# aujxn/faer-amg

Measured on AMD Instinct MI355X. Metric: V-cycles/s + fine-level SpMV GB/s vs HBM peak, 3D 7-pt Laplacian 256³, higher is better.
Workload: dtype f64

## Files before the change

faer-amg_amd/csrc/capi.cpp:

```cpp
#include <atomic>
#include <cmath>
#include <cstring>
#include <string>

#include "handles.hpp"
#include "solve.hpp"

using namespace famg;

namespace {
thread_local std::string g_last_error;
}

amg_status famg::set_last_error(amg_status s, const char *msg) {
    g_last_error = msg;
    return s;
}

namespace {
amg_linop *box(LinOpPtr p) { return new amg_linop{std::move(p)}; }

LinOp &need(const amg_linop *h) {
    FAMG_REQUIRE(h && h->op, AMG_ERR_INVALID, "null amg_linop handle");
    return *h->op;
}

CsrPtr need_csr(const amg_linop *h) {
    need(h);
    auto p = std::dynamic_pointer_cast<CsrOp>(h->op);
    FAMG_REQUIRE(p, AMG_ERR_INVALID, "operator is not a CSR matrix");
    return p;
}

std::shared_ptr<MultigridOp> need_mg(const amg_linop *h) {
    need(h);
    auto p = std::dynamic_pointer_cast<MultigridOp>(h->op);
    FAMG_REQUIRE(p, AMG_ERR_INVALID, "operator is not a multigrid");
    return p;
}

amg_ctx *ctx_of(const LinOp &op) {
    return reinterpret_cast<amg_ctx *>(op.ctx);
}

template <typename F>
void for_columns(LinOp &op, double *out, int64_t ld_out, const double *rhs, int64_t ld_rhs,
                 int64_t k, amg_mem mem, int64_t out_rows, int64_t rhs_rows, F &&f) {
    FAMG_REQUIRE(k >= 0, AMG_ERR_INVALID, "negative column count");
    if (k == 0) return;
    FAMG_REQUIRE(out && rhs, AMG_ERR_INVALID, "null vector");
    FAMG_REQUIRE(ld_out >= out_rows && ld_rhs >= rhs_rows, AMG_ERR_INVALID, "leading dimension too small");
    Ctx &ctx = *op.ctx;
    ctx.set_device();
    if (mem == AMG_MEM_DEVICE) {
        for (int64_t c = 0; c < k; c++) f(out + c * ld_out, rhs + c * ld_rhs);
        return;
    }
    FAMG_REQUIRE(mem == AMG_MEM_HOST, AMG_ERR_INVALID, "bad amg_mem");
    amg_ctx *ac = ctx_of(op);
    if (ac->stage_in.size() < (size_t)rhs_rows) ac->stage_in.resize(rhs_rows);
    if (ac->stage_out.size() < (size_t)out_rows) ac->stage_out.resize(out_rows);
    for (int64_t c = 0; c < k; c++) {
        FAMG_CHECK_HIP(hipMemcpyAsync(ac->stage_in.get(), rhs + c * ld_rhs, rhs_rows * sizeof(double),
                                      hipMemcpyHostToDevice, ctx.stream));
        f(ac->stage_out.get(), ac->stage_in.get());
        FAMG_CHECK_HIP(hipMemcpyAsync(out + c * ld_out, ac->stage_out.get(), out_rows * sizeof(double),
                                      hipMemcpyDeviceToHost, ctx.stream));
        FAMG_CHECK_HIP(hipStreamSynchronize(ctx.stream));
    }
}

}

namespace famg {
void export_plan(const std::vector<LaunchRec> &plan, amg_launch_rec *recs, int64_t cap, int64_t *count) {
    *count = (int64_t)plan.size();
    if (!recs) return;
    for (int64_t i = 0; i < std::min<int64_t>(cap, (int64_t)plan.size()); i++) {
        const LaunchRec &r = plan[i];
        amg_launch_rec &o = recs[i];
        o.level = r.level;
        o.role = r.role;
        o.kernel = r.kernel;
        o.mode = r.mode;
        o.rows = r.rows;
        o.bytes = r.bytes;
        o.csr_bytes = r.csr_bytes;
        std::memset(o.name, 0, sizeof(o.name));
        std::strncpy(o.name, r.name, sizeof(o.name) - 1);
    }
}
}

namespace famg {
static std::atomic<int64_t> g_flag_val[FLAG_COUNT] = {
    {(int64_t)env_is_one("FAMG_FOLD_XSCS")},
    {(int64_t)env_not_zero("FAMG_DIA_DK")},
    {[] {
        const int64_t w = env_int("FAMG_VEC_WPR", 0);
        return (w == 1 || w == 2 || w == 4) ? w : (int64_t)0;
    }()},
    {env_int("FAMG_GTX_TIME", 2)},
    {env_int("FAMG_SGS27_MARCH", 1)},
    {env_int("FAMG_XS_PIPE", 2)},
    {env_int("FAMG_BSR_KERNEL", 0)},
    {env_int("FAMG_BSR_LONG", 48)},
    {env_int("FAMG_DIA7_RP", 0)},
    {env_int("FAMG_FINE_FUSE", 1)},
    {env_int("FAMG_DENSE_TAIL", 4096)},
    {env_int("FAMG_BLOCK_CYCLE", 1)},
    {env_int("FAMG_BLOCK_SMOOTHER_COLS", 1)}};
static std::atomic<uint64_t> g_flag_gen{0};
int64_t flag(FlagId f) { return g_flag_val[f].load(std::memory_order_relaxed); }
void set_flag(FlagId f, int64_t v) {
    g_flag_val[f].store(v);
    g_flag_gen.fetch_add(1);
}
uint64_t flags_generation() { return g_flag_gen.load(); }
}

extern "C" {

const char *amg_last_error(void) { return g_last_error.c_str(); }
const char *amg_version(void) { return "faer-amg_amd 0.1.0 (gfx950)"; }

amg_status amg_ctx_create(int device, void *hip_stream, amg_ctx **out) {
    return guard([&] {
        FAMG_REQUIRE(out, AMG_ERR_INVALID, "null output pointer");
        int ndev = 0;
        FAMG_CHECK_HIP(hipGetDeviceCount(&ndev));
        FAMG_REQUIRE(device >= 0 && device < ndev, AMG_ERR_INVALID, "device index out of range");
        auto *c = new amg_ctx();
        c->ctx.device = device;
        try {
            c->ctx.set_device();
            if (hip_stream) {
                c->ctx.stream = static_cast<hipStream_t>(hip_stream);
            } else {
                FAMG_CHECK_HIP(hipStreamCreateWithFlags(&c->ctx.stream, hipStreamNonBlocking));
                c->ctx.own_stream = true;
            }
            hipDeviceProp_t prop;
            FAMG_CHECK_HIP(hipGetDeviceProperties(&prop, device));
            c->ctx.num_cus = prop.multiProcessorCount;
        } catch (...) {
            delete c;
            throw;
        }
        *out = c;
    });
}

amg_status amg_ctx_destroy(amg_ctx *ctx) {
    return guard([&] {
        if (!ctx) return;
        ctx->ctx.set_device();
        if (ctx->ctx.stream) (void)hipStreamSynchronize(ctx->ctx.stream);
        delete ctx;
    });
}

amg_status amg_ctx_synchronize(amg_ctx *ctx) {
    return guard([&] {
        FAMG_REQUIRE(ctx, AMG_ERR_INVALID, "null context");
        ctx->ctx.set_device();
        FAMG_CHECK_HIP(hipStreamSynchronize(ctx->ctx.stream));
    });
}

amg_status amg_ctx_stream(amg_ctx *ctx, void **hip_stream) {
    return guard([&] {
        FAMG_REQUIRE(ctx && hip_stream, AMG_ERR_INVALID, "null argument");
        *hip_stream = ctx->ctx.stream;
    });
}

amg_status amg_ctx_join_stream(amg_ctx *ctx, void *other, int32_t ctx_waits) {
    return guard([&] {
        FAMG_REQUIRE(ctx, AMG_ERR_INVALID, "null context");
        hipStream_t o = static_cast<hipStream_t>(other);
        if (o == ctx->ctx.stream) return;
        ctx->ctx.set_device();
        if (!ctx->join_event) FAMG_CHECK_HIP(hipEventCreateWithFlags(&ctx->join_event, hipEventDisableTiming));
        if (ctx_waits) {
            FAMG_CHECK_HIP(hipEventRecord(ctx->join_event, o));
            FAMG_CHECK_HIP(hipStreamWaitEvent(ctx->ctx.stream, ctx->join_event, 0));
        } else {
            FAMG_CHECK_HIP(hipEventRecord(ctx->join_event, ctx->ctx.stream));
            FAMG_CHECK_HIP(hipStreamWaitEvent(o, ctx->join_event, 0));
        }
    });
}

amg_status amg_set_alloc_policy(int32_t policy) {
    return guard([&] {
        FAMG_REQUIRE(policy == 0 || policy == 1, AMG_ERR_INVALID, "policy must be 0 or 1");
        FAMG_REQUIRE(policy == 0 || g_alloc_experiment > 0, AMG_ERR_UNSUPPORTED,
                     "contiguous allocations read stale data across kernels on gfx950 (DESIGN.md 3)");
        g_alloc_policy = policy;
    });
}

amg_status amg_set_value_codes(int32_t enable) {
    return guard([&] {
        FAMG_REQUIRE(enable >= 0 && enable <= 2, AMG_ERR_INVALID, "enable must be 0, 1 or 2");
        g_value_codes = enable;
    });
}

amg_status amg_set_sgs_fused(int32_t enable) {
    return guard([&] {
        FAMG_REQUIRE(enable >= 0 && enable <= 2, AMG_ERR_INVALID, "enable must be 0, 1 or 2");
        g_sgs_fused = enable;
    });
}

amg_status amg_sgs_fused(const amg_linop *op, int32_t *fused) {
    return guard([&] {
        FAMG_REQUIRE(fused, AMG_ERR_INVALID, "null output");
        auto p = std::dynamic_pointer_cast<SgsOp>(need(op).shared_from_this());
        FAMG_REQUIRE(p, AMG_ERR_INVALID, "operator is not an SGS smoother");
        *fused = p->fused27 ? 1 : 0;
    });
}

amg_status amg_set_spmv_format(int32_t policy) {
    return guard([&] {
        FAMG_REQUIRE(policy >= 0 && policy <= 3, AMG_ERR_INVALID, "policy must be 0..3");
        g_spmv_format_policy = policy;
    });
}


amg_status amg_csr_create(amg_ctx *ctx, int64_t nrows, int64_t ncols, const int64_t *rowptr,
                          const int64_t *colidx, const double *vals, amg_linop **out) {
    return guard([&] {
        FAMG_REQUIRE(ctx && out, AMG_ERR_INVALID, "null argument");
        FAMG_REQUIRE(nrows >= 0 && ncols >= 0, AMG_ERR_INVALID, "negative dimension");
        ctx->ctx.set_device();
        auto p = make_csr(&ctx->ctx);
        csr_from_host(p->m, &ctx->ctx, nrows, ncols, rowptr, colidx, vals);
        p->nrows = nrows;
        p->ncols = ncols;
        *out = box(p);
    });
}

__attribute__((visibility("default"))) amg_status amg_csr_create_device_i32(
    amg_ctx *ctx, int64_t nrows, int64_t ncols, const int32_t *rowptr, const int32_t *colidx,
    const double *vals, amg_linop **out) {
    return guard([&] {
        FAMG_REQUIRE(ctx && out && rowptr, AMG_ERR_INVALID, "null argument");
        ctx->ctx.set_device();
        hipStream_t s = ctx->ctx.stream;
        std::vector<int32_t> rp32(nrows + 1);
        FAMG_CHECK_HIP(hipMemcpyAsync(rp32.data(), rowptr, (nrows + 1) * sizeof(int32_t), hipMemcpyDeviceToHost, s));
        FAMG_CHECK_HIP(hipStreamSynchronize(s));
        std::vector<int64_t> rp(rp32.begin(), rp32.end());
        const int64_t nnz = rp[nrows];
        auto p = make_csr(&ctx->ctx);
        csr_alloc(p->m, &ctx->ctx, nrows, ncols, nnz);
        FAMG_CHECK_HIP(hipMemcpyAsync(p->m.rp64.get(), rp.data(), (nrows + 1) * sizeof(int64_t), hipMemcpyHostToDevice, s));
        if (nnz) {
            FAMG_CHECK_HIP(hipMemcpyAsync(p->m.col.get(), colidx, nnz * sizeof(int32_t), hipMemcpyDeviceToDevice, s));
// ... 911 lines not shown
```

faer-amg_amd/csrc/common.hpp:

```cpp
#pragma once

#include <hip/hip_runtime.h>

#include <cstdint>
#include <cstdio>
#include <cstdlib>
#include <memory>
#include <stdexcept>
#include <string>
#include <vector>

#include "../../include/amg.h"

namespace famg {

struct AmgError : std::runtime_error {
    amg_status status;
    AmgError(amg_status s, const std::string &msg) : std::runtime_error(msg), status(s) {}
};

[[noreturn]] inline void fail(amg_status s, const std::string &msg) { throw AmgError(s, msg); }

#define FAMG_CHECK_HIP(expr)                                                               \
    do {                                                                                   \
        hipError_t e_ = (expr);                                                            \
        if (e_ != hipSuccess) {                                                            \
            ::famg::fail(e_ == hipErrorOutOfMemory ? AMG_ERR_OOM : AMG_ERR_HIP,            \
                         std::string(#expr) + ": " + hipGetErrorString(e_) + " at " +      \
                             __FILE__ + ":" + std::to_string(__LINE__));                   \
        }                                                                                  \
    } while (0)

#define FAMG_REQUIRE(cond, status, msg)                                                    \
    do {                                                                                   \
        if (!(cond)) ::famg::fail(status, msg);                                            \
    } while (0)

extern int g_alloc_policy;

extern bool g_alloc_debug;

extern int g_alloc_experiment;
inline void *dev_alloc(size_t bytes) {
    void *p = nullptr;
    const bool large = bytes >= (size_t(16) << 20);
    if (g_alloc_policy == 1 && large) {
        if (hipExtMallocWithFlags(&p, bytes, hipDeviceMallocContiguous) == hipSuccess && p) {
            if (g_alloc_debug) fprintf(stderr, "famg alloc contiguous %p %zu\n", p, bytes);
            if (g_alloc_experiment == 2) FAMG_CHECK_HIP(hipDeviceSynchronize());
            return p;
        }
        (void)hipGetLastError();
        p = nullptr;
    }
    FAMG_CHECK_HIP(hipMalloc(&p, bytes));
    if (g_alloc_debug && large) fprintf(stderr, "famg alloc plain %p %zu\n", p, bytes);
    return p;
}

template <typename T> class DevBuf {
  public:
    DevBuf() = default;
    explicit DevBuf(size_t n) { resize(n); }
    DevBuf(const DevBuf &) = delete;
    DevBuf &operator=(const DevBuf &) = delete;
    DevBuf(DevBuf &&o) noexcept : p_(o.p_), n_(o.n_) { o.p_ = nullptr; o.n_ = 0; }
    DevBuf &operator=(DevBuf &&o) noexcept {
        if (this != &o) { release(); p_ = o.p_; n_ = o.n_; o.p_ = nullptr; o.n_ = 0; }
        return *this;
    }
    ~DevBuf() { release(); }
    void resize(size_t n, size_t pad = 0) {
        release();
        if (n + pad) p_ = static_cast<T *>(dev_alloc((n + pad) * sizeof(T)));
        n_ = n;
    }
    void release() {
        if (p_) (void)hipFree(p_);
        p_ = nullptr;
        n_ = 0;
    }
    T *get() const { return p_; }
    size_t size() const { return n_; }
    size_t bytes() const { return n_ * sizeof(T); }

  private:
    T *p_ = nullptr;
    size_t n_ = 0;
};

struct Ctx {
    int device = 0;
    hipStream_t stream = nullptr;
    bool own_stream = false;
    int num_cus = 256;
    DevBuf<double> red_partials;
    DevBuf<double> red_result;
    double *host_red = nullptr;
    void set_device() const { FAMG_CHECK_HIP(hipSetDevice(device)); }
    ~Ctx();
};

inline int64_t ceil_div(int64_t a, int64_t b) { return (a + b - 1) / b; }

inline bool env_is_one(const char *name) {
    const char *e = getenv(name);
    return e && e[0] == '1';
}
inline bool env_not_zero(const char *name) {
    const char *e = getenv(name);
    return !(e && e[0] == '0');
}
inline int64_t env_int(const char *name, int64_t dflt) {
    const char *e = getenv(name);
    return e ? atoll(e) : dflt;
}
inline int env_char(const char *name) {
    const char *e = getenv(name);
    return e ? (int)(unsigned char)e[0] : -1;
}

enum FlagId : int { FLAG_FOLD_XSCS = 0, FLAG_DIA_DK = 1, FLAG_VEC_WPR = 2, FLAG_GTX_TIME = 3, FLAG_SGS27_MARCH = 4, FLAG_XS_PIPE = 5,
              FLAG_BSR_KERNEL = 6, FLAG_BSR_LONG = 7,
              FLAG_DIA7_RP = 8, FLAG_FINE_FUSE = 9, FLAG_DENSE_TAIL = 10, FLAG_BLOCK_CYCLE = 11,
              FLAG_BLOCK_SMOOTHER_COLS = 12, FLAG_COUNT = 13 };
int64_t flag(FlagId f);
void set_flag(FlagId f, int64_t v);
uint64_t flags_generation();

struct LaunchRec {
    int32_t level, role, kernel, mode;
    int64_t rows, bytes, csr_bytes;
    const char *name;
};
struct LaunchLog {
    std::vector<LaunchRec> recs;
    int32_t level = 0, role = AMG_ROLE_OTHER;
    int32_t level_base = 0;
};
extern thread_local LaunchLog *g_launch_log;
struct LaunchLogScope {
    LaunchLog *const saved = g_launch_log;
    explicit LaunchLogScope(LaunchLog *log) { g_launch_log = log; }
    ~LaunchLogScope() { g_launch_log = saved; }
    LaunchLogScope(const LaunchLogScope &) = delete;
    LaunchLogScope &operator=(const LaunchLogScope &) = delete;
};
inline void log_launch(const char *name, int32_t kernel, int32_t mode, int64_t rows, int64_t bytes,
                       int64_t csr_bytes = -1) {
    if (g_launch_log)
        g_launch_log->recs.push_back({g_launch_log->level, g_launch_log->role, kernel, mode, rows, bytes,
                                      csr_bytes < 0 ? bytes : csr_bytes, name});
}
inline void log_at(int64_t level, int32_t role) {
    if (g_launch_log) {
        g_launch_log->level = g_launch_log->level_base + (int32_t)level;
        g_launch_log->role = role;
    }
}

}
```

faer-amg_amd/csrc/sellp.hip:

```cpp
#include <algorithm>
#include <cstdlib>
#include <cstring>
#include <map>

#include "famg.hpp"

namespace famg {

struct SellpArgs {
    const char *vals;
    const int64_t *eoff;
    const int32_t *row0;
    const int2 *pat;
    const int32_t *offs;
    const int32_t *rbase;
    const double *vtab;
    int32_t ntab, slice0, nslices, ncols, w2, spw;
    const double *x;
    double *y;
    const double *b;
    const double *d;
    const uint8_t *dc;
    const double *dt;
    double *y2;
};

template <int MODE> __device__ __forceinline__ double sellp_x(const SellpArgs &a, int c) { return a.x[c]; }

template <int MODE, int L, int U>
__device__ __forceinline__ void sellp_f64(const SellpArgs &a, int64_t e0, const int32_t *__restrict__ off, int w,
                                          int s0, int q, int base, int lane, double &acc) {
    double v[U], xx[U];
#pragma unroll
    for (int u = 0; u < U; u++) {
        const int t = (s0 + u) * L + q;
        const bool in = t < w;
        const int c = min(max(base + off[in ? t : 0], 0), a.ncols - 1);
        const double val = __builtin_nontemporal_load(reinterpret_cast<const double *>(a.vals) + e0 +
                                                      (int64_t)(s0 + u) * 64 + lane);
        v[u] = in ? val : 0.0;
        xx[u] = sellp_x<MODE>(a, c);
    }
#pragma unroll
    for (int u = 0; u < U; u++) acc = fma(v[u], xx[u], acc);
}

template <int MODE, int L, int VB, int W>
__device__ __forceinline__ void sellp_words(const SellpArgs &a, const double *stab, const uint32_t *wp, int k0,
                                            const int32_t *__restrict__ off, int w, int q, int base, double &acc) {
    constexpr int K = 32 / VB;
    uint32_t wd[W];
#pragma unroll
    for (int j = 0; j < W; j++) wd[j] = __builtin_nontemporal_load(wp + (int64_t)(k0 + j) * 64);
    double v[W * K], xx[W * K];
#pragma unroll
    for (int u = 0; u < W * K; u++) {
        const int t = (k0 * K + u) * L + q;
        const bool in = t < w;
        const int c = min(max(base + off[in ? t : 0], 0), a.ncols - 1);
        v[u] = stab[(wd[u / K] >> ((u % K) * VB)) & ((1u << VB) - 1)];
        xx[u] = (L > 1 || in) ? sellp_x<MODE>(a, c) : 0.0;
    }
#pragma unroll
    for (int u = 0; u < W * K; u++) acc = fma(v[u], xx[u], acc);
}

template <int MODE, int L, int VB>
__device__ __forceinline__ void sellp_slice(const SellpArgs &a, const double *stab, int sl) {
    const int s = a.slice0 + sl;
    const int lane = threadIdx.x & 63;
    const int r = lane / L, q = lane % L;
    const int row = a.row0[s] + r;
    const bool live = row < a.row0[s + 1];
    const int rowc = live ? row : a.row0[s];
    const int base = a.rbase ? a.rbase[rowc] : rowc;
    double br = 0.0, xr = 0.0, dr = 0.0, yr = 0.0;
    if (live && q == 0) {
        if constexpr (MODE == SPMV_RESID) br = a.b[row];
        if constexpr (MODE == SPMV_ADD) yr = a.y[row];
        if constexpr (MODE == SPMV_ADD0) yr = (a.dc ? a.dt[a.dc[row]] : a.d[row]) * a.b[row];
        if constexpr (MODE == SPMV_JACOBI) {
            xr = a.x[row];
            br = a.b[row];
            dr = a.dc ? a.dt[a.dc[row]] : a.d[row];
        }
        if constexpr (MODE == SPMV_SETDF) dr = a.dc ? a.dt[a.dc[row]] : a.d[row];
    }
    const int2 pw = a.pat[s];
    const int32_t *off = a.offs + pw.x;
    const int w = pw.y;
    const int S = (w + L - 1) / L;
    const int64_t e0 = a.eoff[s];
    double acc = 0.0;
    if constexpr (VB == 0) {
        int s0 = 0;
        if (a.w2)
            for (; s0 + 8 <= S; s0 += 8) sellp_f64<MODE, L, 8>(a, e0, off, w, s0, q, base, lane, acc);
        for (; s0 + 4 <= S; s0 += 4) sellp_f64<MODE, L, 4>(a, e0, off, w, s0, q, base, lane, acc);
        switch (S - s0) {
        case 1: sellp_f64<MODE, L, 1>(a, e0, off, w, s0, q, base, lane, acc); break;
        case 2: sellp_f64<MODE, L, 2>(a, e0, off, w, s0, q, base, lane, acc); break;
        case 3: sellp_f64<MODE, L, 3>(a, e0, off, w, s0, q, base, lane, acc); break;
        default: break;
        }
    } else {
        constexpr int K = 32 / VB;
        const uint32_t *wp = reinterpret_cast<const uint32_t *>(a.vals) + e0 + lane;
        const int nw = (S + K - 1) / K;
        int k = 0;
        if (a.w2) for (; k + 2 <= nw; k += 2) sellp_words<MODE, L, VB, 2>(a, stab, wp, k, off, w, q, base, acc);
        for (; k < nw; k++) sellp_words<MODE, L, VB, 1>(a, stab, wp, k, off, w, q, base, acc);
    }
#pragma unroll
    for (int m = L / 2; m > 0; m >>= 1) acc += __shfl_xor(acc, m);
    if (live && q == 0) {
        if constexpr (MODE == SPMV_SET) a.y[row] = acc;
        else if constexpr (MODE == SPMV_SETDF) {
            a.y[row] = acc;
            a.y2[row] = dr * acc;
        } else if constexpr (MODE == SPMV_ADD || MODE == SPMV_ADD0) a.y[row] = yr + acc;
        else if constexpr (MODE == SPMV_RESID) a.y[row] = br - acc;
        else a.y[row] = xr + dr * (br - acc);
    }
}

template <int MODE, int L, int VB>
__global__ __launch_bounds__(256) void spmv_sellp_kernel(SellpArgs a) {
    __shared__ double stab[VB ? 256 : 1];
    if constexpr (VB != 0) {
        for (int i = threadIdx.x; i < a.ntab; i += 256) stab[i] = a.vtab[i];
        __syncthreads();
    }
    const int blk = xcd_remap(blockIdx.x, gridDim.x);
    const int wv = __builtin_amdgcn_readfirstlane(blk * 4 + (int)(threadIdx.x >> 6));
    const int s0 = wv * a.spw, s1 = min(s0 + a.spw, a.nslices);
    for (int sl = s0; sl < s1; sl++) sellp_slice<MODE, L, VB>(a, stab, sl);
}

static bool sellp_disabled() {
    static const bool off = env_is_one("FAMG_NO_SELLP");
    return off;
}

bool build_sellp(GpuCsr &m, const std::vector<int64_t> &rp, int64_t other_bytes) {
    if (g_spmv_format_policy != 0 || sellp_disabled() || m.no_sellp || m.nrows < 1024 || m.nnz == 0 ||
        m.ncols < 2)
        return false;
    const int64_t n = m.nrows;
    const bool square = m.nrows == m.ncols;
    std::vector<unsigned long long> tab;
    int vb = csr_value_table(m, tab);
    if (vb == 16) return false;
    const double avg = (double)m.nnz / (double)n;
    if (vb == 0 && m.nnz < 48 * n) return false;
    if (vb != 0 && m.nnz < 16 * n) return false;
    int L = 1;
    while (L < 64 && (n * L) / 64 < 32768 && avg / (2 * L) >= 8) L *= 2;
    if (vb == 0 && L < 2) return false;
    const int R = 64 / L;
    const int K = vb ? 32 / vb : 1;
    hipStream_t st = m.ctx->stream;
    std::vector<int32_t> col(m.nnz);
    FAMG_CHECK_HIP(hipMemcpyAsync(col.data(), m.col.get(), m.nnz * sizeof(int32_t), hipMemcpyDeviceToHost, st));
    FAMG_CHECK_HIP(hipStreamSynchronize(st));
    std::vector<int32_t> base(n);
    for (int64_t i = 0; i < n; i++) {
        int32_t b = square ? (int32_t)i : INT32_MAX;
        if (!square)
            for (int64_t e = rp[i]; e < rp[i + 1]; e++) b = std::min(b, col[e]);
        base[i] = b == INT32_MAX ? 0 : b;
    }
    std::vector<int32_t> row0;
    std::vector<int64_t> seg_slc{0};
    for (size_t g = 0; g + 1 < m.seg_rows.size(); g++) {
        for (int64_t i = m.seg_rows[g]; i < m.seg_rows[g + 1]; i += R) row0.push_back((int32_t)i);
        seg_slc.push_back((int64_t)row0.size());
    }
    row0.push_back((int32_t)n);
    const int64_t ns = (int64_t)row0.size() - 1;
    std::vector<std::vector<int32_t>> pats;
    std::map<std::vector<int32_t>, int32_t> dict;
    std::vector<int32_t> pid(ns);
    std::vector<int64_t> eoff(ns + 1, 0);
    int64_t elems = 0;
    for (int64_t k = 0; k < ns; k++) {
        std::vector<int32_t> u;
        for (int64_t i = row0[k]; i < row0[k + 1]; i++)
            for (int64_t e = rp[i]; e < rp[i + 1]; e++) u.push_back(col[e] - base[i]);
        std::sort(u.begin(), u.end());
        u.erase(std::unique(u.begin(), u.end()), u.end());
        if (u.empty()) u.push_back(0);
        auto it = dict.find(u);
        if (it == dict.end()) {
            it = dict.emplace(u, (int32_t)pats.size()).first;
            pats.push_back(u);
            if ((int64_t)pats.size() > std::max<int64_t>(64, ns / 8)) return false;
        }
        pid[k] = it->second;
        const int64_t S = ((int64_t)u.size() + L - 1) / L;
        eoff[k + 1] = eoff[k] + (vb ? (S + K - 1) / K : S) * 64;
        elems += S * 64;
    }
    if (vb == 0 && (double)elems > 1.3 * (double)m.nnz) return false;
    std::vector<int32_t> poff(pats.size() + 1, 0), offs;
    for (size_t p = 0; p < pats.size(); p++) {
        offs.insert(offs.end(), pats[p].begin(), pats[p].end());
        poff[p + 1] = (int32_t)offs.size();
    }
    const int64_t units = eoff[ns];
    const int64_t meta = (int64_t)(20 * (ns + 1) + 4 * offs.size()) + (square ? 0 : 4 * n);
    const int64_t stream = units * (vb ? 4 : 8) + meta + 8 * (int64_t)tab.size();
    if (vb && (double)stream > 0.5 * (double)other_bytes) return false;
    std::vector<double> val(m.nnz);
    FAMG_CHECK_HIP(hipMemcpyAsync(val.data(), m.val.get(), m.nnz * sizeof(double), hipMemcpyDeviceToHost, st));
    FAMG_CHECK_HIP(hipStreamSynchronize(st));
    std::vector<double> fv;
    std::vector<uint32_t> words;
    int zero_code = 0;
    if (vb) {
        zero_code = (int)(std::lower_bound(tab.begin(), tab.end(), 0ull) - tab.begin());
        uint32_t zw = 0;
        for (int u = 0; u < 32 / vb; u++) zw |= (uint32_t)zero_code << (u * vb);
        words.assign(eoff[ns], zw);
    } else {
        fv.assign(units, 0.0);
    }
    const int KK = vb ? 32 / vb : 1;
#pragma omp parallel for schedule(dynamic, 64)
    for (int64_t k = 0; k < ns; k++) {
        const std::vector<int32_t> &u = pats[pid[k]];
        for (int64_t i = row0[k]; i < row0[k + 1]; i++) {
            const int r = (int)(i - row0[k]);
            for (int64_t e = rp[i]; e < rp[i + 1]; e++) {
                const int32_t o = col[e] - base[i];
                const size_t t = (size_t)(std::lower_bound(u.begin(), u.end(), o) - u.begin());
                const int64_t s = (int64_t)(t / L), lane = (int64_t)r * L + (int64_t)(t % L);
                if (vb == 0) {
                    fv[eoff[k] + s * 64 + lane] = val[e];
                } else {
                    unsigned long long bits;
                    std::memcpy(&bits, &val[e], 8);
                    const uint32_t c = (uint32_t)(std::lower_bound(tab.begin(), tab.end(), bits) - tab.begin());
                    uint32_t &wd = words[eoff[k] + (s / KK) * 64 + lane];
                    const int sh = (int)(s % KK) * vb;
                    wd = (wd & ~(((1u << vb) - 1) << sh)) | (c << sh);
                }
            }
        }
    }
    m.sellp.vbits = vb;
    if (vb) {
        m.sellp.vals.resize(std::max<int64_t>(16, (int64_t)words.size() * 4));
        FAMG_CHECK_HIP(hipMemcpyAsync(m.sellp.vals.get(), words.data(), words.size() * 4, hipMemcpyHostToDevice, st));
        m.sellp.vtab.resize(tab.size());
        FAMG_CHECK_HIP(hipMemcpyAsync(m.sellp.vtab.get(), tab.data(), tab.size() * 8, hipMemcpyHostToDevice, st));
        m.sellp.ntab = (int64_t)tab.size();
    } else {
        m.sellp.vals.resize(std::max<int64_t>(16, units * 8));
        FAMG_CHECK_HIP(hipMemcpyAsync(m.sellp.vals.get(), fv.data(), units * 8, hipMemcpyHostToDevice, st));
        m.sellp.ntab = 0;
    }
    if (!square) {
        m.sellp.rbase.resize(n);
        FAMG_CHECK_HIP(hipMemcpyAsync(m.sellp.rbase.get(), base.data(), n * 4, hipMemcpyHostToDevice, st));
    }
    m.sellp.eoff.resize(ns + 1);
    m.sellp.row0.resize(ns + 1);
    std::vector<int32_t> pat(2 * std::max<int64_t>(1, ns), 0);
    for (int64_t k = 0; k < ns; k++) {
        pat[2 * k] = poff[pid[k]];
        pat[2 * k + 1] = poff[pid[k] + 1] - poff[pid[k]];
    }
    m.sellp.pat.resize(pat.size());
    m.sellp.offs.resize(std::max<size_t>(1, offs.size()));
    FAMG_CHECK_HIP(hipMemcpyAsync(m.sellp.eoff.get(), eoff.data(), (ns + 1) * 8, hipMemcpyHostToDevice, st));
    FAMG_CHECK_HIP(hipMemcpyAsync(m.sellp.row0.get(), row0.data(), (ns + 1) * 4, hipMemcpyHostToDevice, st));
    FAMG_CHECK_HIP(hipMemcpyAsync(m.sellp.pat.get(), pat.data(), pat.size() * 4, hipMemcpyHostToDevice, st));
    FAMG_CHECK_HIP(hipMemcpyAsync(m.sellp.offs.get(), offs.data(), offs.size() * 4, hipMemcpyHostToDevice, st));
    FAMG_CHECK_HIP(hipStreamSynchronize(st));
    m.sellp.slices = ns;
    m.sellp.elems = vb ? eoff[ns] * (32 / vb) : units;
    m.sellp.L = L;
    m.sellp.seg_slc = seg_slc;
    m.sellp.meta_bytes = meta;
    m.sellp.stream = (vb ? eoff[ns] * 4 : units * 8) + meta + 8 * m.sellp.ntab;
    return true;
}

static int sellp_w2_enabled() {
    static const int on = env_is_one("FAMG_SELLP_W1") ? 0 : 1;
    return on;
}

static int sellp_spw() {
    static const int k = (int)env_int("FAMG_SELLP_SPW", 1), v = k > 0 ? k : 1;
    return v;
}

void spmv_sellp(const GpuCsr &m, const double *x, double *y, SpmvMode mode, const SpmvEpi &epi, hipStream_t s,
                int64_t seg) {
    const int64_t s0 = seg < 0 ? 0 : m.sellp.seg_slc[seg];
    const int64_t s1 = seg < 0 ? m.sellp.slices : m.sellp.seg_slc[seg + 1];
    if (s1 <= s0) return;
    SellpArgs a{m.sellp.vals.get(), m.sellp.eoff.get(), m.sellp.row0.get(),
                reinterpret_cast<const int2 *>(m.sellp.pat.get()), m.sellp.offs.get(), m.sellp.rbase.get(), m.sellp.vtab.get(), (int32_t)m.sellp.ntab,
                (int32_t)s0, (int32_t)(s1 - s0), (int32_t)m.ncols, sellp_w2_enabled(), sellp_spw(), x, y, epi.b, epi.d, epi.dc, epi.dt,
                epi.y2};
    FAMG_REQUIRE(mode != SPMV_SETDF || (epi.y2 && (epi.d || epi.dc)), AMG_ERR_INVALID, "SETDF needs y2 and d");
    const dim3 grid((unsigned)ceil_div(s1 - s0, 4 * (int64_t)a.spw)), block(256);
#define FAMG_SELLP(L, VB)                                                                          \
    switch (mode) {                                                                                \
    case SPMV_SET: spmv_sellp_kernel<SPMV_SET, L, VB><<<grid, block, 0, s>>>(a); break;            \
    case SPMV_ADD: spmv_sellp_kernel<SPMV_ADD, L, VB><<<grid, block, 0, s>>>(a); break;            \
    case SPMV_RESID: spmv_sellp_kernel<SPMV_RESID, L, VB><<<grid, block, 0, s>>>(a); break;        \
    case SPMV_JACOBI: spmv_sellp_kernel<SPMV_JACOBI, L, VB><<<grid, block, 0, s>>>(a); break;      \
    case SPMV_ADD0: spmv_sellp_kernel<SPMV_ADD0, L, VB><<<grid, block, 0, s>>>(a); break;          \
    case SPMV_SETDF: spmv_sellp_kernel<SPMV_SETDF, L, VB><<<grid, block, 0, s>>>(a); break;        \
    default: fail(AMG_ERR_UNSUPPORTED, "pattern SELL: unsupported SpMV epilogue");                 \
    }
#define FAMG_SELLP_VB(L)                                                                           \
    if (m.sellp.vbits == 0) { FAMG_SELLP(L, 0) }                                                   \
    else if (m.sellp.vbits == 4) { FAMG_SELLP(L, 4) }                                              \
    else { FAMG_SELLP(L, 8) }
    switch (m.sellp.L) {
    case 1: FAMG_SELLP_VB(1) break;
    case 2: FAMG_SELLP_VB(2) break;
    case 4: FAMG_SELLP_VB(4) break;
    case 8: FAMG_SELLP_VB(8) break;
    case 16: FAMG_SELLP_VB(16) break;
    case 32: FAMG_SELLP_VB(32) break;
    default: FAMG_SELLP_VB(64) break;
    }
#undef FAMG_SELLP_VB
#undef FAMG_SELLP
    FAMG_CHECK_HIP(hipGetLastError());
}

}
```

faer-amg_amd/faer_amg_amd/__init__.py:

```python
from __future__ import annotations

import ctypes as C
import os

import numpy as np

_PKG_DIR = os.path.dirname(os.path.abspath(__file__))
LIB_PATH = os.environ.get("FAMG_LIB") or os.path.join(os.path.dirname(_PKG_DIR), "libfaer_amg_amd.so")

if not os.path.exists(LIB_PATH):
    raise ImportError(
        f"{LIB_PATH} not found: build the HIP library first "
        "(python -c 'import __graft_entry__ as g; g.build()' or make -C faer-amg_amd)")

_lib = C.CDLL(LIB_PATH)


def source_hash(root=None):
    import glob
    import hashlib
    root = root or os.path.dirname(_PKG_DIR)
    src = os.path.join(root, "csrc")
    files = []
    for pat in ("*.hip", "*.cpp", "*.hpp", "*.inc"):
# ... 349 lines not shown
        return self.dims()[1]

    def apply(self, out, rhs):
        po, mo, no, ko, lo = _dptr(out)
        pr, mr, nr, kr, lr = _dptr(rhs)
        if mo != mr or ko != kr:
            raise ValueError("out and rhs must live in the same memory with equal columns")
        with _ordered(self.ctx, mo):
            _ck(_lib.amg_linop_apply(self.h, po, lo, pr, lr, ko, mo))
        return out

    def transpose_apply(self, out, rhs):
        po, mo, no, ko, lo = _dptr(out)
        pr, mr, nr, kr, lr = _dptr(rhs)
        with _ordered(self.ctx, mo):
            _ck(_lib.amg_linop_transpose_apply(self.h, po, lo, pr, lr, ko, mo))
        return out

    def apply_in_place(self, rhs):
        p, m, n, k, ld = _dptr(rhs)
        with _ordered(self.ctx, m):
            _ck(_lib.amg_precond_apply_in_place(self.h, p, ld, k, m))
        return rhs

    def transpose_apply_in_place(self, rhs):
        p, m, n, k, ld = _dptr(rhs)
        with _ordered(self.ctx, m):
            _ck(_lib.amg_precond_transpose_apply_in_place(self.h, p, ld, k, m))
        return rhs

    def __matmul__(self, x):
        x = np.ascontiguousarray(x, np.float64)
        out = np.zeros(self.nrows)
        return self.apply(out, x)


class SparseMatOp(LinOp):

    @classmethod
    def from_arrays(cls, ctx, nrows, ncols, rowptr, col, val):
        rp = np.ascontiguousarray(rowptr, np.int64)
        ci = np.ascontiguousarray(col, np.int64)
        va = np.ascontiguousarray(val, np.float64)
        h = vp()
        _ck(_lib.amg_csr_create(ctx.h, int(nrows), int(ncols), rp.ctypes.data_as(vp),
                                ci.ctypes.data_as(vp), va.ctypes.data_as(vp), C.byref(h)))
        return cls(h, ctx)

    @classmethod
    def from_scipy(cls, ctx, M):
        M = M.tocsr()
        M.sort_indices()
        return cls.from_arrays(ctx, M.shape[0], M.shape[1], M.indptr, M.indices, M.data)

    @classmethod
    def laplace3d_7pt(cls, ctx, nx, ny, nz):
        h = vp()
        _ck(_lib.amg_gen_laplace3d_7pt(ctx.h, nx, ny, nz, C.byref(h)))
        return cls(h, ctx)

    @classmethod
    def aniso27(cls, ctx, nx, ny, nz, ex=1.0, ey=1.0, ez=0.01):
        h = vp()
        _ck(_lib.amg_gen_aniso27(ctx.h, nx, ny, nz, ex, ey, ez, C.byref(h)))
        return cls(h, ctx)

    @classmethod
    def random7(cls, ctx, nx, ny, nz, seed=42, window=4096):
        h = vp()
        _ck(_lib.amg_gen_random_7pt(ctx.h, nx, ny, nz, seed, window, C.byref(h)))
        return cls(h, ctx)

    @property
    def nnz(self):
        v = i64()
        _ck(_lib.amg_csr_nnz(self.h, C.byref(v)))
        return v.value

    def spmv_info(self):
        info = np.zeros(8, np.int64)
        _ck(_lib.amg_csr_spmv_info(self.h, info.ctypes.data_as(vp)))
        keys = ("kernel", "stream_bytes", "csr_bytes", "slices", "stored_entries",
                "slices_implicit", "slices_u16", "slices_i32")
        d = dict(zip(keys, (int(v) for v in info)))
        d["kernel"] = ("csr-stream", "sell", "vector", "dia", "bsr", "sellp", "classes", "xsell", "gtc")[d["kernel"]]
        vc = np.zeros(2, np.int64)
        _ck(_lib.amg_csr_value_codes(self.h, vc.ctypes.data_as(vp)))
        d["value_bits"], d["value_table"] = int(vc[0]), int(vc[1])
        dr = np.zeros(4, np.int64)
        _ck(_lib.amg_csr_dia_range(self.h, dr.ctypes.data_as(vp)))
        d["dia_rows"] = (int(dr[0]), int(dr[1]))
        d["dia_diagonals"], d["dia_bits"] = int(dr[2]), int(dr[3])
        ci = np.zeros(4, np.int64)
        _ck(_lib.amg_csr_class_info(self.h, ci.ctypes.data_as(vp)))
        d["classes"], d["class_offsets"], d["class_id_bits"] = int(ci[0]), int(ci[1]), int(ci[2])
        g = np.zeros(13, np.int64)
        _ck(_lib.amg_csr_grid_info(self.h, g.ctypes.data_as(vp)))
        d["grid"] = tuple(int(v) for v in g[:3])
        d["grid_source"] = ("none", "given", "inferred")[int(g[10])]
        d["gtc"] = ("none", "P", "R", "P", "R")[int(g[11])]
        d["gtc_kind"] = ("none", "gtc", "gtc", "gtx", "gtx")[int(g[11])]
        d["xstaged"] = bool(g[3])
        if d["xstaged"]:
            d["tile"], d["halo"] = tuple(int(v) for v in g[4:7]), tuple(int(v) for v in g[7:10])
            d["tile_source"] = ("none", "table", "timed", "env", "rule")[int(g[12])]
        rl = i64()
        _ck(_lib.amg_csr_row_lanes(self.h, C.byref(rl)))
        d["row_lanes"] = rl.value
        return d

    def spmv_epilogue(self, mode, x, y, b=None, d=None):
        m = {"set": 0, "add": 1, "resid": 2, "jacobi": 3}[mode]
        ptr = lambda t: None if t is None else vp(t.data_ptr())
        with _ordered(self.ctx, AMG_MEM_DEVICE):
            _ck(_lib.amg_csr_spmv_epilogue(self.h, m, ptr(x), ptr(y), ptr(b), ptr(d)))

    def spmm_epilogue(self, mode, X, Y, B=None, d=None):
        m = {"set": 0, "add": 1, "resid": 2, "jacobi": 3}[mode]
        px, _, _, k, ldx = _dptr(X)
        py, _, _, ky, ldy = _dptr(Y)
        if k != ky:
            raise ValueError("X and Y must have equal columns")
        pb, ldb = (None, 0) if B is None else (_dptr(B)[0], _dptr(B)[4])
        with _ordered(self.ctx, AMG_MEM_DEVICE):
            _ck(_lib.amg_csr_spmm_epilogue(self.h, m, px, ldx, py, ldy, pb, ldb,
                                           None if d is None else vp(d.data_ptr()), k))

    def set_grid(self, nx, ny, nz):
        _ck(_lib.amg_csr_set_grid(self.h, nx, ny, nz))

    def arrays(self):
        m, n = self.dims()
        nnz = self.nnz
        rp = np.zeros(m + 1, np.int64)
        ci = np.zeros(max(nnz, 1), np.int64)
        va = np.zeros(max(nnz, 1), np.float64)
        _ck(_lib.amg_csr_download(self.h, rp.ctypes.data_as(vp), ci.ctypes.data_as(vp),
                                  va.ctypes.data_as(vp)))
        return rp, ci[:nnz], va[:nnz]

    def to_scipy(self):
        import scipy.sparse as sp
        rp, ci, va = self.arrays()
        return sp.csr_matrix((va, ci, rp), shape=self.dims())


def csr_spmm_epilogue(A, mode, X, Y, B=None, d=None):
    A.spmm_epilogue(mode, X, Y, B, d)


FLAGS = {"fold_xscs": 0, "dia_dk": 1, "vec_wpr": 2, "gtx_time": 3, "sgs27_march": 4, "xs_pipe": 5, "bsr_kernel": 6,
         "bsr_long": 7,
         "dia7_rp": 8, "fine_fuse": 9, "dense_tail": 10, "block_cycle": 11,
         "block_smoother_cols": 12}


def set_flag(name, value):
    _ck(_lib.amg_set_flag(FLAGS[name], int(value)))


def get_flag(name):
    v = i64()
    _ck(_lib.amg_get_flag(FLAGS[name], C.byref(v)))
    return v.value


def grid_from_offsets(offsets, n):
    o = np.ascontiguousarray(np.asarray(offsets, dtype=np.int64))
    g = np.zeros(3, np.int64)
    found = C.c_int32(0)
    _ck(_lib.amg_grid_from_offsets(o.ctypes.data_as(vp), len(o), int(n), g.ctypes.data_as(vp), C.byref(found)))
    return tuple(int(v) for v in g) if found.value else None


def _wrap(h, ctx, cls=LinOp, refs=()):
    return cls(h, ctx, refs)


def new_jacobi(A, omega=0.66):
    h = vp()
    _ck(_lib.amg_jacobi_create(A.h, omega, C.byref(h)))
    return _wrap(h, A.ctx)


def new_l1(A):
    h = vp()
    _ck(_lib.amg_l1_create(A.h, C.byref(h)))
    return _wrap(h, A.ctx)


def new_l2(A):
    h = vp()
    _ck(_lib.amg_l2_create(A.h, C.byref(h)))
    return _wrap(h, A.ctx)


def diag(ctx, d):
    d = np.ascontiguousarray(d, np.float64)
    h = vp()
    _ck(_lib.amg_diag_create(ctx.h, len(d), d.ctypes.data_as(vp), C.byref(h)))
    return _wrap(h, ctx)


class SymGaussSeidel(LinOp):
    def __init__(self, A, colors=None):
        h = vp()
        cp = None
        if colors is not None:
            colors = np.ascontiguousarray(colors, np.int32)
            cp = colors.ctypes.data_as(vp)
        _ck(_lib.amg_sgs_create(A.h, cp, C.byref(h)))
        super().__init__(h, A.ctx)

    @property
    def ncolors(self):
        v = i64()
        _ck(_lib.amg_sgs_ncolors(self.h, C.byref(v)))
        return v.value

    def sweep_storage(self):
        return sgs_info(self)


def sgs_info(S):
    info = np.zeros(4, np.int64)
    _ck(_lib.amg_sgs_info(S.h, info.ctypes.data_as(vp)))
    return {"colors": int(info[0]), "kernel": ("csr-stream", "sell", "vector", "dia", "bsr", "sellp")[int(info[1])],
            "diagonals": int(info[2]), "bits": int(info[3])}


def set_sgs_fused(enable):
    _ck(_lib.amg_set_sgs_fused(int(enable)))


def sgs_fused(S):
    v = i32()
    _ck(_lib.amg_sgs_fused(S.h, C.byref(v)))
    return bool(v.value)


class ChebyshevConfig(C.Structure):
    _fields_ = [("steps", i64), ("eig_iters", i64), ("eig_ratio", dbl), ("boost", dbl), ("lambda_max", dbl)]

    def __init__(self, **kw):
        super().__init__()
        _ck(_lib.amg_chebyshev_config_default(C.byref(self)))
        for k, v in kw.items():
            setattr(self, k, v)


def new_chebyshev(A, steps=2, eig_ratio=20.0, eig_iters=10, boost=1.1, lambda_max=0.0):
    cfg = ChebyshevConfig(steps=steps, eig_ratio=eig_ratio, eig_iters=eig_iters, boost=boost, lambda_max=lambda_max)
    h = vp()
    _ck(_lib.amg_chebyshev_create(A.h, C.byref(cfg), C.byref(h)))
    return _wrap(h, A.ctx)


def chebyshev_info(S):
    info = np.zeros(6, np.float64)
    _ck(_lib.amg_chebyshev_info(S.h, info.ctypes.data_as(vp)))
    return {"lambda_max": float(info[0]), "lambda_min": float(info[1]), "steps": int(info[2]),
            "ritz": float(info[3]), "row_sum_bound": float(info[4]), "eig_iters": int(info[5])}


def CoarseCholesky(A):
    h = vp()
    _ck(_lib.amg_coarse_chol_create(A.h, C.byref(h)))
    return _wrap(h, A.ctx)


class Multigrid(LinOp):

    def __init__(self, op, smoother, _handle=None):
        if _handle is None:
            h = vp()
            _ck(_lib.amg_multigrid_create(op.h, smoother.h, C.byref(h)))
        else:
            h = _handle
        super().__init__(h, op.ctx)

    @classmethod
    def _from_handle(cls, h, ctx):
        obj = cls.__new__(cls)
        LinOp.__init__(obj, h, ctx)
        return obj

    def add_level(self, op, smoother, r, p):
        _ck(_lib.amg_multigrid_add_level(self.h, op.h, smoother.h, r.h, p.h))
        return self

    def with_cycle_type(self, mu):
        self._mu = mu
        _ck(_lib.amg_multigrid_set(self.h, mu, getattr(self, "_steps", 1)))
        return self

    def with_smoothing_steps(self, steps):
        self._steps = steps
        _ck(_lib.amg_multigrid_set(self.h, getattr(self, "_mu", 1), steps))
        return self

    def set_graph(self, enable):
        _ck(_lib.amg_multigrid_set_graph(self.h, 1 if enable else 0))

    def set_reorder(self, mode):
        _ck(_lib.amg_multigrid_set_option(self.h, 5, int(mode)))

    def run_level(self, l):
# ... 1007 lines not shown
```

Measured before the change: 2611.

## Add software-pipelined chained SELL-P SpMV kernel for small unquantized grids

Adds a new SELL-P SpMV kernel that processes each slice in chunks of C=8 sub-slices. It prefetches the next chunk's column offsets while the current values and x-gathers are in flight, and uses sched_barriers and nontemporal value loads to keep memory requests overlapped. The kernel is selected by default when values are unquantized, L>1, and the grid fits within the resident wave budget, so it mainly targets coarse AMG levels where latency dominates. It adds a new flag, more template instantiations, and tighter launch bounds that could raise register pressure.

```diff
diff --git a/faer-amg_amd/csrc/capi.cpp b/faer-amg_amd/csrc/capi.cpp
--- a/faer-amg_amd/csrc/capi.cpp
+++ b/faer-amg_amd/csrc/capi.cpp
@@ -109,7 +109,8 @@
     {env_int("FAMG_FINE_FUSE", 1)},
     {env_int("FAMG_DENSE_TAIL", 4096)},
     {env_int("FAMG_BLOCK_CYCLE", 1)},
-    {env_int("FAMG_BLOCK_SMOOTHER_COLS", 1)}};
+    {env_int("FAMG_BLOCK_SMOOTHER_COLS", 1)},
+    {env_int("FAMG_SELLP_CHAIN", 1)}};
 static std::atomic<uint64_t> g_flag_gen{0};
 int64_t flag(FlagId f) { return g_flag_val[f].load(std::memory_order_relaxed); }
 void set_flag(FlagId f, int64_t v) {
diff --git a/faer-amg_amd/csrc/common.hpp b/faer-amg_amd/csrc/common.hpp
--- a/faer-amg_amd/csrc/common.hpp
+++ b/faer-amg_amd/csrc/common.hpp
@@ -123,7 +123,7 @@
 enum FlagId : int { FLAG_FOLD_XSCS = 0, FLAG_DIA_DK = 1, FLAG_VEC_WPR = 2, FLAG_GTX_TIME = 3, FLAG_SGS27_MARCH = 4, FLAG_XS_PIPE = 5,
               FLAG_BSR_KERNEL = 6, FLAG_BSR_LONG = 7,
               FLAG_DIA7_RP = 8, FLAG_FINE_FUSE = 9, FLAG_DENSE_TAIL = 10, FLAG_BLOCK_CYCLE = 11,
-              FLAG_BLOCK_SMOOTHER_COLS = 12, FLAG_COUNT = 13 };
+              FLAG_BLOCK_SMOOTHER_COLS = 12, FLAG_SELLP_CHAIN = 13, FLAG_COUNT = 14 };
 int64_t flag(FlagId f);
 void set_flag(FlagId f, int64_t v);
 uint64_t flags_generation();
diff --git a/faer-amg_amd/csrc/sellp.hip b/faer-amg_amd/csrc/sellp.hip
--- a/faer-amg_amd/csrc/sellp.hip
+++ b/faer-amg_amd/csrc/sellp.hip
@@ -124,6 +124,108 @@
     }
 }
 
+
+template <int L, int C>
+__device__ __forceinline__ void sellp_chain_offs(const int32_t *__restrict__ off, int w, int s0, int q, int (&o)[C]) {
+#pragma unroll
+    for (int u = 0; u < C; u++) {
+        const int t0 = (s0 + u) * L;
+        o[u] = off[q < w - t0 ? t0 + q : 0];
+    }
+}
+
+template <int MODE, int L, int C, int N, bool MORE, class Mid>
+__device__ __forceinline__ void sellp_chain_chunk(const SellpArgs &a, const double *__restrict__ vp,
+                                                  const int32_t *__restrict__ off, int w, int s0, int q, int base0,
+                                                  int rb, int (&o)[C], double &acc, Mid &&mid) {
+    double v[N], xx[N];
+#pragma unroll
+    for (int u = 0; u < N; u++) v[u] = __builtin_nontemporal_load(vp + (int64_t)(s0 + u) * 64);
+    __builtin_amdgcn_sched_barrier(0);
+    const int base = base0 + (a.rbase ? rb : 0);
+#pragma unroll
+    for (int u = 0; u < N; u++) xx[u] = sellp_x<MODE>(a, min(max(base + o[u], 0), a.ncols - 1));
+    mid();
+    if constexpr (MORE) sellp_chain_offs<L, C>(off, w, s0 + C, q, o);
+    __builtin_amdgcn_sched_barrier(0);
+#pragma unroll
+    for (int u = 0; u < N; u++) acc = fma(q < w - (s0 + u) * L ? v[u] : 0.0, xx[u], acc);
+}
+
+template <int MODE, int L, int C, int N, class Mid>
+__device__ __forceinline__ void sellp_chain_tail(const SellpArgs &a, const double *__restrict__ vp,
+                                                 const int32_t *__restrict__ off, int w, int s0, int n, int q,
+                                                 int base0, int rb, int (&o)[C], double &acc, Mid &&mid) {
+    if constexpr (N > 0) {
+        if (n == N) sellp_chain_chunk<MODE, L, C, N, false>(a, vp, off, w, s0, q, base0, rb, o, acc, mid);
+        else sellp_chain_tail<MODE, L, C, N - 1>(a, vp, off, w, s0, n, q, base0, rb, o, acc, mid);
+    }
+}
+
+template <int MODE, int L, int C>
+__device__ __forceinline__ void sellp_slice_chain(const SellpArgs &a, int sl) {
+    const int s = a.slice0 + sl;
+    int lane = threadIdx.x & 63;
+    asm volatile("" : "+v"(lane));
+    const int r = lane / L, q = lane % L;
+    const int row = a.row0[s] + r;
+    const bool live = row < a.row0[s + 1];
+    const int rowc = live ? row : a.row0[s];
+    const int2 pw = a.pat[s];
+    const int32_t *off = a.offs + pw.x;
+    const int w = pw.y;
+    const int S = (w + L - 1) / L;
+    const int64_t e0 = a.eoff[s];
+    const double *vp = reinterpret_cast<const double *>(a.vals) +
+                       (((int64_t)__builtin_amdgcn_readfirstlane((int)(e0 >> 32)) << 32) |
+                        (uint32_t)__builtin_amdgcn_readfirstlane((int)e0)) + lane;
+    __builtin_amdgcn_sched_barrier(0);
+    const int base0 = a.rbase ? 0 : rowc;
+    const int rb = *(a.rbase ? a.rbase + rowc : a.row0);
+    int o[C];
+    sellp_chain_offs<L, C>(off, w, 0, q, o);
+    __builtin_amdgcn_sched_barrier(0);
+    double br = 0.0, xr = 0.0, dr = 0.0, yr = 0.0;
+    uint8_t dcode = 0;
+    constexpr bool HAS_D = MODE == SPMV_ADD0 || MODE == SPMV_JACOBI || MODE == SPMV_SETDF;
+    if (live && q == 0) {
+        if constexpr (MODE == SPMV_RESID || MODE == SPMV_ADD0 || MODE == SPMV_JACOBI) br = a.b[row];
+        if constexpr (MODE == SPMV_ADD) yr = a.y[row];
+        if constexpr (MODE == SPMV_JACOBI) xr = a.x[row];
+        if constexpr (HAS_D) {
+            if (a.dc) dcode = a.dc[row];
+            else dr = a.d[row];
+        }
+    }
+    __builtin_amdgcn_sched_barrier(0);
+    double acc = 0.0;
+    auto none = [] {};
+    auto diag = [&] {
+        if constexpr (HAS_D)
+            if (a.dc && live && q == 0) dr = a.dt[dcode];
+    };
+    int s0 = 0;
+    if (S > C) {
+        sellp_chain_chunk<MODE, L, C, C, true>(a, vp, off, w, 0, q, base0, rb, o, acc, diag);
+        for (s0 = C; s0 + C < S; s0 += C) sellp_chain_chunk<MODE, L, C, C, true>(a, vp, off, w, s0, q, base0, rb, o, acc, none);
+        sellp_chain_tail<MODE, L, C, C>(a, vp, off, w, s0, S - s0, q, base0, rb, o, acc, none);
+    } else {
+        sellp_chain_tail<MODE, L, C, C>(a, vp, off, w, 0, S, q, base0, rb, o, acc, diag);
+    }
+#pragma unroll
+    for (int m = L / 2; m > 0; m >>= 1) acc += __shfl_xor(acc, m);
+    if (live && q == 0) {
+        if constexpr (MODE == SPMV_SET) a.y[row] = acc;
+        else if constexpr (MODE == SPMV_SETDF) {
+            a.y[row] = acc;
+            a.y2[row] = dr * acc;
+        } else if constexpr (MODE == SPMV_ADD) a.y[row] = yr + acc;
+        else if constexpr (MODE == SPMV_ADD0) a.y[row] = dr * br + acc;
+        else if constexpr (MODE == SPMV_RESID) a.y[row] = br - acc;
+        else a.y[row] = xr + dr * (br - acc);
+    }
+}
+
 template <int MODE, int L, int VB>
 __global__ __launch_bounds__(256) void spmv_sellp_kernel(SellpArgs a) {
     __shared__ double stab[VB ? 256 : 1];
@@ -135,6 +237,14 @@
     const int wv = __builtin_amdgcn_readfirstlane(blk * 4 + (int)(threadIdx.x >> 6));
     const int s0 = wv * a.spw, s1 = min(s0 + a.spw, a.nslices);
     for (int sl = s0; sl < s1; sl++) sellp_slice<MODE, L, VB>(a, stab, sl);
+}
+
+template <int MODE, int L, int C>
+__global__ __launch_bounds__(256, C <= 8 ? 5 : C <= 16 ? 4 : 2) void spmv_sellp_chain_kernel(SellpArgs a) {
+    const int blk = xcd_remap(blockIdx.x, gridDim.x);
+    const int wv = __builtin_amdgcn_readfirstlane(blk * 4 + (int)(threadIdx.x >> 6));
+    const int s0 = wv * a.spw, s1 = min(s0 + a.spw, a.nslices);
+    for (int sl = s0; sl < s1; sl++) sellp_slice_chain<MODE, L, C>(a, sl);
 }
 
 static bool sellp_disabled() {
@@ -292,6 +402,8 @@
     return on;
 }
 
+constexpr int SELLP_CHAIN_C = 8;
+
 static int sellp_spw() {
     static const int k = (int)env_int("FAMG_SELLP_SPW", 1), v = k > 0 ? k : 1;
     return v;
@@ -308,29 +420,38 @@
                 epi.y2};
     FAMG_REQUIRE(mode != SPMV_SETDF || (epi.y2 && (epi.d || epi.dc)), AMG_ERR_INVALID, "SETDF needs y2 and d");
     const dim3 grid((unsigned)ceil_div(s1 - s0, 4 * (int64_t)a.spw)), block(256);
-#define FAMG_SELLP(L, VB)                                                                          \
+    const int64_t fc = m.sellp.vbits == 0 && m.sellp.L > 1 ? flag(FLAG_SELLP_CHAIN) : 0;
+    const int64_t resident = 4 * 5 * (int64_t)std::max(m.ctx ? m.ctx->num_cus : 256, 1);
+    const bool chain = fc == 2 || (fc != 0 && 4 * (int64_t)grid.x <= resident);
+#define FAMG_SELLP_MODES(KERNEL, L, X)                                                             \
     switch (mode) {                                                                                \
-    case SPMV_SET: spmv_sellp_kernel<SPMV_SET, L, VB><<<grid, block, 0, s>>>(a); break;            \
-    case SPMV_ADD: spmv_sellp_kernel<SPMV_ADD, L, VB><<<grid, block, 0, s>>>(a); break;            \
-    case SPMV_RESID: spmv_sellp_kernel<SPMV_RESID, L, VB><<<grid, block, 0, s>>>(a); break;        \
-    case SPMV_JACOBI: spmv_sellp_kernel<SPMV_JACOBI, L, VB><<<grid, block, 0, s>>>(a); break;      \
-    case SPMV_ADD0: spmv_sellp_kernel<SPMV_ADD0, L, VB><<<grid, block, 0, s>>>(a); break;          \
-    case SPMV_SETDF: spmv_sellp_kernel<SPMV_SETDF, L, VB><<<grid, block, 0, s>>>(a); break;        \
+    case SPMV_SET: KERNEL<SPMV_SET, L, X><<<grid, block, 0, s>>>(a); break;                        \
+    case SPMV_ADD: KERNEL<SPMV_ADD, L, X><<<grid, block, 0, s>>>(a); break;                        \
+    case SPMV_RESID: KERNEL<SPMV_RESID, L, X><<<grid, block, 0, s>>>(a); break;                    \
+    case SPMV_JACOBI: KERNEL<SPMV_JACOBI, L, X><<<grid, block, 0, s>>>(a); break;                  \
+    case SPMV_ADD0: KERNEL<SPMV_ADD0, L, X><<<grid, block, 0, s>>>(a); break;                      \
+    case SPMV_SETDF: KERNEL<SPMV_SETDF, L, X><<<grid, block, 0, s>>>(a); break;                    \
     default: fail(AMG_ERR_UNSUPPORTED, "pattern SELL: unsupported SpMV epilogue");                 \
     }
-#define FAMG_SELLP_VB(L)                                                                           \
-    if (m.sellp.vbits == 0) { FAMG_SELLP(L, 0) }                                                   \
+#define FAMG_SELLP(L, VB) FAMG_SELLP_MODES(spmv_sellp_kernel, L, VB)
+#define FAMG_SELLP_CH(L)                                                                           \
+    if (chain) { FAMG_SELLP_MODES(spmv_sellp_chain_kernel, L, SELLP_CHAIN_C) }                     \
+    else
+#define FAMG_SELLP_VB(L, CHAINED)                                                                  \
+    CHAINED if (m.sellp.vbits == 0) { FAMG_SELLP(L, 0) }                                           \
     else if (m.sellp.vbits == 4) { FAMG_SELLP(L, 4) }                                              \
     else { FAMG_SELLP(L, 8) }
     switch (m.sellp.L) {
-    case 1: FAMG_SELLP_VB(1) break;
-    case 2: FAMG_SELLP_VB(2) break;
-    case 4: FAMG_SELLP_VB(4) break;
-    case 8: FAMG_SELLP_VB(8) break;
-    case 16: FAMG_SELLP_VB(16) break;
-    case 32: FAMG_SELLP_VB(32) break;
-    default: FAMG_SELLP_VB(64) break;
-    }
+    case 1: FAMG_SELLP_VB(1, ) break;
+    case 2: FAMG_SELLP_VB(2, FAMG_SELLP_CH(2)) break;
+    case 4: FAMG_SELLP_VB(4, FAMG_SELLP_CH(4)) break;
+    case 8: FAMG_SELLP_VB(8, FAMG_SELLP_CH(8)) break;
+    case 16: FAMG_SELLP_VB(16, FAMG_SELLP_CH(16)) break;
+    case 32: FAMG_SELLP_VB(32, FAMG_SELLP_CH(32)) break;
+    default: FAMG_SELLP_VB(64, FAMG_SELLP_CH(64)) break;
+    }
+#undef FAMG_SELLP_CH
+#undef FAMG_SELLP_MODES
 #undef FAMG_SELLP_VB
 #undef FAMG_SELLP
     FAMG_CHECK_HIP(hipGetLastError());
diff --git a/faer-amg_amd/faer_amg_amd/__init__.py b/faer-amg_amd/faer_amg_amd/__init__.py
--- a/faer-amg_amd/faer_amg_amd/__init__.py
+++ b/faer-amg_amd/faer_amg_amd/__init__.py
@@ -525,7 +525,7 @@
 FLAGS = {"fold_xscs": 0, "dia_dk": 1, "vec_wpr": 2, "gtx_time": 3, "sgs27_march": 4, "xs_pipe": 5, "bsr_kernel": 6,
          "bsr_long": 7,
          "dia7_rp": 8, "fine_fuse": 9, "dense_tail": 10, "block_cycle": 11,
-         "block_smoother_cols": 12}
+         "block_smoother_cols": 12, "sellp_chain": 13}
 
 
 def set_flag(name, value):
```

New measurement: 2616, median of 4. No clear change (+0.2%).
